# sotelo/parrot

Measured on AMD Instinct MI355X. Metric: acoustic feature frames/sec (train fwd+bwd+allreduce+clip/Adam), higher is better.
Workload: dtype f32; 1 GPU; BASELINE configs[1]: 2-layer attention-GRU decoder, h=1024, batch=64 per GPU, T_enc=200, T_dec=800, fp32; cell=gru, layers=2, hidden=1024, batch_per_gpu=64, global_batch=64, T_enc=200, T_dec=800, parallelism=dp1, params=13919212

## Files before the change

include/parrot_hip.h:

```cpp
#ifndef PARROT_HIP_H
#define PARROT_HIP_H

#include <stddef.h>
#include <stdint.h>

#ifdef __cplusplus
extern "C" {
#endif

#define PARROT_ERR_BADARG 10001
#define PARROT_ERR_UNSUPPORTED 10002

#define PARROT_NORM_EPS 1e-5f
#define PARROT_MAX_LAYERS 3

const char* parrot_hip_version(void);

int parrot_profile_begin(void);
long long parrot_profile_end(double* total_us, double* flops, double* bytes);
long long parrot_profile_end2(double* total_us, double* flops, double* bytes, double* plain4);

#define PARROT_PRECISION_F32 0
#define PARROT_PRECISION_BF16 1
#define PARROT_PRECISION_BF16X3 2
// ... 130 lines not shown
    const float* Wg_f[PARROT_MAX_LAYERS];
    const float* Wc_f[PARROT_MAX_LAYERS];
    const float* Wg_r[PARROT_MAX_LAYERS];
    const float* Wc_r[PARROT_MAX_LAYERS];
    int* att_sup;
    float* persist_ws;
    long long persist_ws_floats;
    float* dh_b[PARROT_MAX_LAYERS];
    float* dhup_b[PARROT_MAX_LAYERS];
    float* dw_b;
    float* dw0_b;
    float* dhup_c[PARROT_MAX_LAYERS];
    float* dw_c;
    float* dw0_c;
    void* dG16[PARROT_MAX_LAYERS];
} ParrotDecoderDesc;

long long parrot_decoder_persist_floats(const ParrotDecoderDesc* desc);
int parrot_decoder_is_persistent(void* plan);
int parrot_decoder_schedule(void* plan);
int parrot_decoder_backward_tick(void* plan);
long long parrot_decoder_trace(void* plan, int which, long long* out, long long cap);
long long parrot_decoder_trace_jobs(void* plan, int which, long long* out, long long cap);
int parrot_decoder_status(void* plan);

int parrot_decoder_create(const ParrotDecoderDesc* desc, void** plan);
int parrot_decoder_writes_bf16_grads(void* plan);
int parrot_decoder_seq_fwd(void* plan, void* stream);
int parrot_decoder_seq_bwd(void* plan, void* stream);
int parrot_decoder_destroy(void* plan);

#define PARROT_READOUT_MAX_SEG 4
typedef struct ParrotReadoutComposedDesc {
    long long M;
    long long ws_floats;
    int nseg, R, O, zero_rows;
    int slice_rows, nbias;
    int K[PARROT_READOUT_MAX_SEG];
    int ldx[PARROT_READOUT_MAX_SEG];
    int lddx[PARROT_READOUT_MAX_SEG];
    int ldwr, ldwo, ldp, lddp;
    int ldgwr, ldgwo;
    const float* x[PARROT_READOUT_MAX_SEG];
    const float* Wr; const float* Wo;
    const float* rb[PARROT_READOUT_MAX_SEG];
    const float* bo;
// ... 196 lines not shown
```

parrot_amd/_lib.py:

```python
from __future__ import annotations

import ctypes as C
import os

from .utils import env_str

_HERE = os.path.dirname(os.path.abspath(__file__))
LIB_PATH = os.path.join(_HERE, "libparrot_hip.so")

MAX_LAYERS = 3

c_float_p = C.c_void_p


class HipLibraryMissing(RuntimeError):
    pass


class HipCallError(RuntimeError):
    pass


class GruSeqDesc(C.Structure):
    _fields_ = [
# ... 170 lines not shown
    "parrot_label_gather": (_i, [C.POINTER(LabelTablesDesc), _vp]),
    "parrot_label_segsum_ws_floats": (C.c_longlong, [_ll, _i, _i]),
    "parrot_label_segsum": (_i, [C.POINTER(LabelTablesDesc), _vp, _ll, _vp]),
    "parrot_gru_seq_create": (_i, [C.POINTER(GruSeqDesc), C.POINTER(C.c_void_p)]),
    "parrot_gru_seq_fwd": (_i, [_vp, _vp]),
    "parrot_gru_seq_bwd": (_i, [_vp, _vp]),
    "parrot_gru_seq_destroy": (_i, [_vp]),
    "parrot_gru_seq_route": (_i, [_vp, C.POINTER(C.c_int)]),
    "parrot_gru_seq_rowwise_supported": (_i, [_i, _i, _i, _i]),
    "parrot_lstm_seq_create": (_i, [C.POINTER(LstmSeqDesc), C.POINTER(C.c_void_p)]),
    "parrot_lstm_seq_fwd": (_i, [_vp, _vp]),
    "parrot_lstm_seq_bwd": (_i, [_vp, _vp]),
    "parrot_lstm_seq_destroy": (_i, [_vp]),
    "parrot_gmm_attention_fwd": (_i, [_vp] * 10 + [_i] * 6 + [_f] * 4 + [_vp]),
    "parrot_gmm_attention_bwd": (_i, [_vp] * 10 + [_i] * 6 + [_f, _vp]),
    "parrot_decoder_create": (_i, [C.POINTER(DecoderDesc), C.POINTER(C.c_void_p)]),
    "parrot_decoder_persist_floats": (C.c_longlong, [C.POINTER(DecoderDesc)]),
    "parrot_decoder_is_persistent": (_i, [_vp]),
    "parrot_decoder_schedule": (_i, [_vp]),
    "parrot_decoder_backward_tick": (_i, [_vp]),
    "parrot_decoder_writes_bf16_grads": (_i, [_vp]),
    "parrot_decoder_trace": (C.c_longlong, [_vp, _i, C.POINTER(C.c_longlong), C.c_longlong]),
    "parrot_decoder_trace_jobs": (C.c_longlong, [_vp, _i, C.POINTER(C.c_longlong), C.c_longlong]),
    "parrot_decoder_seq_fwd": (_i, [_vp, _vp]),
    "parrot_decoder_seq_bwd": (_i, [_vp, _vp]),
    "parrot_decoder_destroy": (_i, [_vp]),
    "parrot_readout_composed_ws_floats": (C.c_longlong, [C.POINTER(ReadoutComposedDesc)]),
    "parrot_readout_composed_fwd": (_i, [C.POINTER(ReadoutComposedDesc), _vp, _vp]),
    "parrot_readout_composed_bwd": (_i, [C.POINTER(ReadoutComposedDesc), _vp, _vp]),
    "parrot_sample_create": (_i, [C.POINTER(SampleDesc), C.POINTER(C.c_void_p)]),
    "parrot_sample_persist_floats": (C.c_longlong, [C.POINTER(SampleDesc)]),
    "parrot_sample_is_persistent": (_i, [_vp]),
    "parrot_sample_is_bf16": (_i, [_vp]),
    "parrot_sample_plan_pieces_dry": (_i, [C.POINTER(SampleDesc), _i, C.POINTER(C.c_int)]),
    "parrot_sample_plan_digest_dry": (_i, [C.POINTER(SampleDesc), _i, C.POINTER(C.c_ulonglong)]),
    "parrot_sample_status": (_i, [_vp]),
    "parrot_sample_stops_early": (_i, [_vp]),
    "parrot_sample_steps_run": (_i, [_vp, C.POINTER(C.c_int)]),
    "parrot_decoder_status": (_i, [_vp]),
    "parrot_sample_run": (_i, [_vp, _vp]),
    "parrot_sample_destroy": (_i, [_vp]),
    "parrot_plan_last_error": (_i, [_vp]),
    "parrot_sumsq": (_i, [_vp, _sz, _vp, _vp]),
    "parrot_tile_weights": (_i, [_vp, _i, _i, _i, _vp, _i, _i, _vp]),
    "parrot_tile_weights_bf16": (_i, [_vp, _i, _i, _i, _vp, _i, _i, _vp]),
    "parrot_set_gemm_precision": (_i, [_i]),
# ... 54 lines not shown
```

parrot_amd/build.py:

```python
from __future__ import annotations

import hashlib
import os
import subprocess
import sys
from concurrent.futures import ThreadPoolExecutor

from .utils import env_str

HERE = os.path.dirname(os.path.abspath(__file__))
CSRC = os.path.join(HERE, "csrc")
OUT = os.path.join(HERE, "libparrot_hip.so")
OBJDIR = os.path.join(CSRC, "build")
ARCH = "gfx950"

SOURCES = ["skinny.hip", "biggemm.hip", "attention.hip", "elementwise.hip", "quantize.hip",
           "plans.hip", "plans_decode.hip", "capi.hip", "samplernn.hip", "persist.hip", "sr_persist.hip", "rowgru.hip", "trainops.hip", "readout.hip",
           "gmmcost.hip", "labeltables.hip"]
EXTRA_FLAGS = {"quantize.hip": ["-ffp-contract=off"]}
if env_str("PARROT_PM_DEPTH"):
    EXTRA_FLAGS["persist.hip"] = ["-DPM_DEPTH=" + env_str("PARROT_PM_DEPTH")]


def _hipcc() -> str:
    for cand in (os.environ.get("HIPCC"), "/opt/rocm/bin/hipcc", "hipcc"):
        if cand and (os.path.isabs(cand) and os.path.exists(cand) or not os.path.isabs(cand)):
            return cand
    return "hipcc"


def _digest(paths) -> str:
    h = hashlib.sha256()
    for p in sorted(paths):
        with open(p, "rb") as f:
            h.update(p.encode())
            h.update(f.read())
    return h.hexdigest()


def build(force: bool = False, verbose: bool = True, timers: bool = False) -> str:
    global OUT, OBJDIR
    if timers:
# ... 41 lines not shown
```

parrot_amd/csrc/plans.hip:

```cpp
#include "pm_builder.h"
#include "switches.h"

namespace {

struct GruSeqPlan : PlanBase {
    ParrotGruSeqDesc d;

    bool rowwise = false;
    int reason = PARROT_GRU_ROUTE_SHAPE;
    int waves = 4;
    float* tiled = nullptr;
    ~GruSeqPlan() override {
        if (tiled) (void)hipFree(tiled);
    }
    int launch_path(int why) {
        rowwise = false;
        reason = why;
        return 0;
    }
    int setup_rowwise() {
        if (!rowgru_supported(d.T, d.B, d.H, d.nchain)) return launch_path(PARROT_GRU_ROUTE_SHAPE);
        if (env_int("PARROT_GRU_ROWWISE", 1) == 0) return launch_path(PARROT_GRU_ROUTE_SWITCH);
        for (int ch = 0; ch < d.nchain; ++ch)
            if (!d.Wg[ch] || !d.Wc[ch] || ((uintptr_t)d.Wg[ch] & 15) || ((uintptr_t)d.Wc[ch] & 15))
// ... 178 lines not shown
    bool persist_ok = false;
    PmProgram pm_prog;

    ~DecoderPlan() override {
        if (att_flags && !flags_fake) (void)hipFree(att_flags);
        if (bwd_flags && !flags_fake) (void)hipFree(bwd_flags);
    }

    int run(int which, hipStream_t s) override {
        BgPrecisionScope precision(d.bf16 ? 1 : -1);
        return PlanBase::run(which, s);
    }

    int enqueue(int which, hipStream_t s) override {
        BgPrecisionScope precision(d.bf16 ? 1 : -1);
        if (which == 0 && persist_ok) return pm_launch(pm_prog, s);
        if (schedule == 3) return which == 0 ? fwd_skew(s) : bwd_skew(s);
        if (which == 1 && bwd_hetero && (schedule == 0 || schedule == 5)) return bwd8(s);
        if (schedule == 5) return which == 0 ? fwd5(s) : bwd(s);
        if (schedule == 7) return which == 0 ? fwd7(s) : bwd(s);
        return which == 0 ? fwd(s) : bwd(s);
    }

    int trace(int which, std::vector<TraceRec>& out, std::vector<TraceJob>* jobs_out = nullptr) {
        if (persist_ok || (schedule != 0 && schedule < 5) || d.layer_norm) return PARROT_ERR_UNSUPPORTED;
        Tracer tr;
        g_tracer = &tr;
        const int rc = enqueue(which, nullptr);
        g_tracer = nullptr;
        out.swap(tr.recs);
        if (jobs_out) jobs_out->swap(tr.jobs);
        return rc;
    }

    int krows(int l) const { return d.H + d.E + l * d.H; }
    float* dctx(float* of_l0, float* of_upper, int l, int t) const {
        const size_t BE = (size_t)d.B * d.E;
        return l == 0 ? of_l0 + (size_t)t * BE : of_upper + (size_t)(t + 1) * BE;
    }
    SkSeg fseg(const float* A, int lda, int l, int g, int r0, int K, int ldw) const {
        if (tiled) {
            const float* Wt = g == 0 ? d.Wg_f[l] : d.Wc_f[l];
            if (d.bf16) return sk_seg(A, lda, Wt + (size_t)(r0 >> 5) * 256, (krows(l) >> 5) * 256, K, 3);
            return sk_seg(A, lda, Wt + (size_t)(r0 >> 4) * 256, (krows(l) >> 4) * 256, K, 2);
        }
        const float* W = g == 0 ? d.Wg[l] : d.Wc[l];
        return sk_seg(A, lda, W + (size_t)r0 * ldw, ldw, K, 0);
    }
    SkSeg rseg(const float* A, int l, int g, int r0, int ldw) const {
        if (tiled) {
            const float* Wt = g == 0 ? d.Wg_r[l] : d.Wc_r[l];
            if (d.bf16) return sk_seg(A, ldw, Wt + (size_t)(r0 >> 4) * (ldw >> 5) * 256, (ldw >> 5) * 256, ldw, 3);
            return sk_seg(A, ldw, Wt + (size_t)(r0 >> 4) * (ldw >> 4) * 256, (ldw >> 4) * 256, ldw, 2);
        }
// ... 926 lines not shown
int parrot_decoder_schedule(void* plan) { return plan ? static_cast<DecoderPlan*>(plan)->schedule : -1; }
int parrot_decoder_backward_tick(void* plan) { return plan ? (static_cast<DecoderPlan*>(plan)->bwd_hetero ? 8 : (static_cast<DecoderPlan*>(plan)->bwd_fused ? 7 : 0)) : -1; }
int parrot_decoder_writes_bf16_grads(void* plan) {
    const DecoderPlan* p = static_cast<const DecoderPlan*>(plan);
    if (!p || !p->bwd_fused) return 0;
    for (int l = 0; l < p->d.L; ++l)
        if (!p->d.dG16[l]) return 0;
    return 1;
}
long long parrot_decoder_trace_jobs(void* plan, int which, long long* out, long long cap) { PH_ENTRY();
    if (!plan || which < 0 || which > 1) return -PARROT_ERR_BADARG;
    std::vector<TraceRec> recs;
    std::vector<TraceJob> jobs;
    const int rc = static_cast<DecoderPlan*>(plan)->trace(which, recs, &jobs);
    if (rc != 0) return -(long long)rc;
    const long long n = (long long)jobs.size();
    if (out)
        for (long long i = 0; i < n && i < cap; ++i) {
            out[6 * i] = jobs[i].launch; out[6 * i + 1] = jobs[i].job; out[6 * i + 2] = jobs[i].M;
            out[6 * i + 3] = jobs[i].N; out[6 * i + 4] = jobs[i].Kmax_seg_sum; out[6 * i + 5] = jobs[i].epi;
        }
    return n;
}
long long parrot_decoder_trace(void* plan, int which, long long* out, long long cap) { PH_ENTRY();
    if (!plan || which < 0 || which > 1) return -PARROT_ERR_BADARG;
    std::vector<TraceRec> recs;
    const int rc = static_cast<DecoderPlan*>(plan)->trace(which, recs);
    if (rc != 0) return -(long long)rc;
    const long long n = (long long)recs.size();
    if (out)
        for (long long i = 0; i < n && i < cap; ++i) {
            out[5 * i] = recs[i].launch; out[5 * i + 1] = recs[i].job; out[5 * i + 2] = recs[i].kind;
            out[5 * i + 3] = recs[i].lo; out[5 * i + 4] = recs[i].hi;
        }
    return n;
}

int parrot_decoder_seq_fwd(void* plan, void* stream) { PH_ENTRY(); return static_cast<PlanBase*>(plan)->run(0, (hipStream_t)stream); }
int parrot_decoder_seq_bwd(void* plan, void* stream) { PH_ENTRY(); return static_cast<PlanBase*>(plan)->run(1, (hipStream_t)stream); }
int parrot_decoder_destroy(void* plan) { PH_ENTRY();
    delete static_cast<PlanBase*>(plan);
    return 0;
}

int parrot_plan_last_error(void* plan) { PH_ENTRY(); return plan ? static_cast<PlanBase*>(plan)->last_error : PARROT_ERR_BADARG; }

// ... 2 lines not shown
```

parrot_amd/csrc/plans_common.h:

```cpp
#pragma once
#include <stdlib.h>
#include <string.h>
#include <algorithm>
#include <array>
#include <memory>
#include <new>
#include <vector>
#include "../../include/parrot_hip.h"
#include "attention.h"
#include "biggemm.h"
#include "elementwise.h"
#include "persist.h"
#include "rowgru.h"
#include "skinny.h"

namespace {


struct PlanBase {
    int last_error = 0;
    int use_graph = 0;
    hipGraphExec_t exec[2] = {nullptr, nullptr};
    hipStream_t cap_stream = nullptr;
    virtual ~PlanBase() {
// ... 23 lines not shown
            e = hipGraphInstantiate(&exec[which], graph, nullptr, nullptr, 0);
            hipGraphDestroy(graph);
            if (e != hipSuccess) {
                exec[which] = nullptr;
                return note((int)e);
            }
        }
        return note((int)hipGraphLaunch(exec[which], s));
    }
    int note(int rc) {
        if (rc != 0 && last_error == 0) last_error = rc;
        return rc;
    }
};

#define PL_TRY(x)                \
    do {                         \
        const int rc__ = (x);    \
        if (rc__ != 0) return rc__; \
    } while (0)

struct TraceRec { long long launch, job, kind, lo, hi; };
struct TraceJob { long long launch, job, M, N, Kmax_seg_sum, epi; };
struct Tracer {
    std::vector<TraceRec> recs;
    std::vector<TraceJob> jobs;
    long long launch = -1;
    void begin() { ++launch; }
    void mat(const void* p, long long rows, long long cols, long long ld, int kind, int job, int elt = 4) {
        if (!p || rows < 1 || cols < 1) return;
        const long long base = (long long)(uintptr_t)p;
        if (ld == cols) { recs.push_back({launch, job, kind, base, base + rows * cols * elt}); return; }
        for (long long r = 0; r < rows; ++r) recs.push_back({launch, job, kind, base + r * ld * elt, base + (r * ld + cols) * elt});
    }
    void sk_job(const SkJob& j, int id) {
        long long ks = 0;
        for (int q = 0; q < j.nseg; ++q) ks += j.seg[q].K;
        jobs.push_back({launch, id, j.M, j.N, ks, j.epi});
        for (int q = 0; q < j.nseg; ++q)
            mat(j.seg[q].A, j.M, j.seg[q].K, j.seg[q].lda, (j.wait_flag && (j.wait_all || q == j.nseg - 1)) ? 3 : 0, id);
        mat(j.add, j.M, j.N, j.ld_add, 0, id);
        const int H = j.H;
        switch (j.epi) {
            case SK_EPI_LINEAR:
                mat(j.out, j.M, j.N, j.ldo, j.accumulate ? 2 : 1, id);
                if (j.ksplit > 1) mat(j.o1, j.M, j.N, j.ldo1, j.ldo2 ? 2 : 1, id);
                if (j.ksplit > 2) mat(j.kout2, j.M, j.N, j.ldo1, 1, id);
                if (j.ksplit > 3) mat(j.kout3, j.M, j.N, j.ldo1, 1, id);
                break;
            case SK_EPI_GRU_GATES:
                mat(j.e0, j.M, H, j.lde0, 0, id); mat(j.o1, j.M, H, j.ldo1, 1, id); mat(j.o2, j.M, H, j.ldo2, 1, id);
// ... 37 lines not shown
    }
    void chain(const LstmStateBwdChain& c, int B, int H, int id) {
        mat(c.dh, B, H, H, 0, id); mat(c.dh2, B, H, H, 0, id); mat(c.dh3, B, H, H, 0, id); mat(c.dh4, B, H, H, 0, id);
        mat(c.dh5, B, H, H, 0, id); mat(c.dh6, B, H, H, 0, id);
        mat(c.gates, B, 4 * H, 4 * H, 0, id);
        mat(c.c_prev, B, H, H, 0, id); mat(c.c_new, B, H, H, 0, id);
        mat(c.dc, B, H, H, 2, id); mat(c.dP, B, 4 * H, 4 * H, 1, id);
        mat(c.dP16, B, 4 * H, 4 * H, 1, id, 2);
    }
};
thread_local Tracer* g_tracer = nullptr;
enum { TRACE_JOB_ATT = 100, TRACE_JOB_CHAIN = 200 };

int launch_jobs(const SkJob* jobs, int n, hipStream_t s, int full_wgs = 0, int force_tile = 0, int force_wide = 0) {
    SkLaunch L;
    PL_TRY(sk_make_launch(L, jobs, n));
    L.force_wide = force_wide;
    if (g_tracer) {
        g_tracer->begin();
        for (int q = 0; q < n; ++q) {
            if (jobs[q].wait_flag) return PARROT_ERR_BADARG;
            g_tracer->sk_job(jobs[q], q);
        }
        return 0;
    }
    L.full_wgs = full_wgs;
    L.force_tile = force_tile;
    return sk_launch(L, s);
}

int traced_att_fwd_launch(const AttFwdArgs& att, hipStream_t s) {
    if (g_tracer) {
        g_tracer->begin();
        g_tracer->att_fwd(att, TRACE_JOB_ATT);
        return 0;
    }
    return att_fwd_launch(att, s);
}

int launch_jobs_att(const SkJob* jobs, int n, const AttFwdArgs& att, hipStream_t s, int full_wgs = 0) {
    if (n < 1) return traced_att_fwd_launch(att, s);
    SkLaunch L;
    PL_TRY(sk_make_launch(L, jobs, n));
    if (g_tracer) {
        g_tracer->begin();
        g_tracer->att_fwd(att, TRACE_JOB_ATT);
// ... 129 lines not shown
```

parrot_amd/csrc/skinny.h:

```cpp
#pragma once
#include "common.h"

#ifndef SK_NWAVES
#define SK_NWAVES 8
#endif
enum { SK_MAXSEG = 5, SK_MAXJOB = 9, SK_NW = SK_NWAVES, SK_THREADS = SK_NW * 64 };

enum SkEpi {
    SK_EPI_LINEAR = 0,
    SK_EPI_GRU_GATES = 1,
    SK_EPI_GRU_CAND = 2,
    SK_EPI_BWD_RH = 3,
    SK_EPI_LSTM = 4,
};

enum SkAct { SK_ACT_NONE = 0, SK_ACT_RELU = 1, SK_ACT_TANH = 2, SK_ACT_SIGMOID = 3 };

struct SkSeg {
    const float* A;
    const float* B;
    int lda, ldb, K, b_kcontig;
};

struct SkJob {
    SkSeg seg[SK_MAXSEG];
    int nseg, M, N, epi;
    int act, accumulate, H, aligned;
    const float* bias;
    const float* add;
// ... 2 lines not shown
    const float* e1;
    float* o1;
    float* o2;
    const float* mask;
    int ld_add, ldo, lde0, lde1, ldo1, ldo2, wait_all, ksplit;
    float* kout2;
    float* kout3;
    const unsigned* wait_flag;
    unsigned wait_target;
    int colmode;
};

struct SkLaunch {
    SkJob job[SK_MAXJOB];
    int njobs, zmode;
    int tile_end[SK_MAXJOB];
    int force_tile;
    int force_wide;
    int full_wgs;
};

int sk_launch(const SkLaunch& L, hipStream_t stream);
void sk_prepare(const SkLaunch& Lin, SkLaunch& L, dim3& grid, size_t& lds, int& mbnb);
struct AttFwdArgs;
int sk_launch_att(const SkLaunch& L, const AttFwdArgs& att, hipStream_t stream);
struct AttBwdArgs;
struct GruStateBwdArgs;
int sk_launch_bwd_hetero(const SkLaunch& L, const AttBwdArgs* att, const GruStateBwdArgs& sa, int l0_chain, hipStream_t stream);
struct LstmStateBwdArgs;
int sk_launch_bwd_fused(const SkLaunch& L, const AttBwdArgs* att, const LstmStateBwdArgs& sa, int l0_chain,
                        unsigned* const* flags, hipStream_t stream);
int sk_zero_words_launch(unsigned* p, int n, hipStream_t stream);
void sk_profile_begin();
long long sk_profile_end(double* total_us, double* flops, double* bytes);
long long sk_profile_end2(double* total_us, double* flops, double* bytes, double* plain);

static inline SkSeg sk_seg(const float* A, int lda, const float* B, int ldb, int K, int b_kcontig) {
    SkSeg s;
    s.A = A; s.B = B; s.lda = lda; s.ldb = ldb; s.K = K; s.b_kcontig = b_kcontig;
    return s;
}
int sk_tile_weights_launch(const float* W, int rows, int cols, int ld, float* out, int mode, int lstm_H,
                           hipStream_t stream);
int sk_tile_weights_bf16_launch(const float* W, int rows, int cols, int ld, void* out, int mode, int lstm_H,
                                hipStream_t stream);
void sk_job_init(SkJob& j);
// ... 5 lines not shown
```

parrot_amd/csrc/skinny.hip:

```cpp
#include "skinny.h"
#include "att_fwd_body.h"
#include "att_bwd_body.h"
#include "elementwise.h"
#include "switches.h"

#include <stdio.h>
#include <stdlib.h>

#include <hip/hip_ext.h>
#include <string.h>
#include <type_traits>
#include <vector>

template <bool AL>
__device__ __forceinline__ f32x4 ld4k(const float* __restrict__ p, int k, int K) {
    f32x4 v = {0.f, 0.f, 0.f, 0.f};
    if (AL) {
        if (k < K) v = *reinterpret_cast<const f32x4*>(p);
    } else {
#pragma unroll
        for (int u = 0; u < 4; ++u)
            if (k + u < K) v[u] = p[u];
    }
    return v;
// ... 130 lines not shown
        __builtin_amdgcn_s_sleep(8);
        if ((++it & 1023u) == 0 && wall_clock64() - t0 > 100000000ull) __builtin_trap();
    }
    __builtin_amdgcn_fence(__ATOMIC_ACQUIRE, "workgroup");
    asm volatile("" ::: "memory");
}
__device__ __forceinline__ __amdgpu_buffer_rsrc_t sk_rsrc(const void* p) {
    const unsigned long long a = (unsigned long long)p;
    const unsigned lo = __builtin_amdgcn_readfirstlane((unsigned)a);
    const unsigned hi = __builtin_amdgcn_readfirstlane((unsigned)(a >> 32));
    void* q = (void*)(((unsigned long long)hi << 32) | lo);
    return __builtin_amdgcn_make_buffer_rsrc(q, 0, 0x7fffffff, 0x00020000);
}

#ifdef SK_TIMERS
__constant__ unsigned long long* sk_timer_buf = nullptr;
#define SK_STAMP(i)                                                                                                  \
    do {                                                                                                             \
        if (sk_timer_buf && (threadIdx.x & 63) == 0) {                                                               \
            const size_t wg_ = blockIdx.x + (size_t)gridDim.x * (blockIdx.y + (size_t)gridDim.y * blockIdx.z);       \
            sk_timer_buf[(wg_ * 16 + (threadIdx.x >> 6)) * 8 + (i)] = wall_clock64();                                \
        }                                                                                                            \
    } while (0)
#else
#define SK_STAMP(i) do { } while (0)
#endif

__device__ __forceinline__ unsigned sk_off(int m, int ld, int c) { return __umul24((unsigned)m, (unsigned)ld) + (unsigned)c; }

template <int MB, int NB, bool FAST>
__device__ __forceinline__ void sk_body(const SkJob& job, int tile0, f32x4* red) {
    const int tid = threadIdx.x;
    const int lane = tid & 63;
    const int wave = __builtin_amdgcn_readfirstlane(tid >> 6);
    const int kk = lane >> 4, i = lane & 15;
    const int m0 = blockIdx.y * (16 * MB);
    const int M = job.M, N = job.N;
    SK_STAMP(0);
    asm volatile("" ::"s"(job.M), "s"(job.N), "s"(job.epi), "s"(job.H), "s"(job.nseg), "s"(job.accumulate), "s"(job.colmode),
                 "s"(job.bias), "s"(job.add), "s"(job.out), "s"(job.e0), "s"(job.e1), "s"(job.o1), "s"(job.ld_add),
                 "s"(job.ldo), "s"(job.lde0), "s"(job.lde1), "s"(job.ldo1), "s"(job.wait_flag), "s"(job.seg[0].A),
                 "s"(job.seg[0].B), "s"(job.seg[0].lda), "s"(job.seg[0].ldb), "s"(job.seg[0].K), "s"(job.seg[0].b_kcontig),
                 "s"(job.seg[1].A), "s"(job.seg[1].B), "s"(job.seg[1].lda), "s"(job.seg[1].ldb), "s"(job.seg[1].K));
    if (m0 >= M) return;

    f32x4 acc[MB][NB];
#pragma unroll
    for (int rb = 0; rb < MB; ++rb)
#pragma unroll
        for (int nb = 0; nb < NB; ++nb) acc[rb][nb] = (f32x4){0.f, 0.f, 0.f, 0.f};

    constexpr int NBLK = MB * NB;
    constexpr int EG = (SK_NW % NBLK == 0) ? (SK_NW / NBLK > 4 ? 4 : SK_NW / NBLK) : 1;
    constexpr int RPW = 4 / EG, EWAVES = NBLK * EG;
    const int eblk = wave % NBLK, er0 = (wave / NBLK) * RPW;
    float p_bias = 0.f, p_add[RPW], p_e0[RPW], p_e1[RPW], p_oc[RPW];
#pragma unroll
    for (int r = 0; r < RPW; ++r) p_add[r] = p_e0[r] = p_e1[r] = p_oc[r] = 0.f;
    const bool has_add = job.add != nullptr;
    if (wave < EWAVES) {
        const int rb_ = eblk / NB, tile_ = tile0 + eblk % NB;
// ... 26 lines not shown
            p_oc[r] = q_oc[sk_off(m, l_oc, c_oc)];
        }
    }

    SK_STAMP(6);
    if (FAST) {
        int cend[SK_MAXSEG], slda[SK_MAXSEG], sldb[SK_MAXSEG];
        const float* sA[SK_MAXSEG];
        const float* sB[SK_MAXSEG];
        int total = 0;
        const int csh = job.seg[0].b_kcontig == 3 ? 5 : 4;
        const bool flagged = job.wait_flag != nullptr;
        const int nsm = flagged ? job.nseg - 1 : job.nseg;
#pragma unroll
        for (int s = 0; s < SK_MAXSEG; ++s) {
            const bool on = s < nsm;
            const int ss = on ? s : 0;
            if (on) total += job.seg[ss].K >> csh;
            cend[s] = total;
            sA[s] = job.seg[ss].A; sB[s] = job.seg[ss].B; slda[s] = job.seg[ss].lda; sldb[s] = job.seg[ss].ldb;
        }
        int mrow[MB], ncl[NB], btile[NB];
#pragma unroll
        for (int rb = 0; rb < MB; ++rb) mrow[rb] = min(m0 + rb * 16 + ((lane >> 2) & 15), M - 1);
#pragma unroll
        for (int nb = 0; nb < NB; ++nb) {
            ncl[nb] = min(sk_jcol(job, tile0 + nb, i), N - 1);
            btile[nb] = min(tile0 + nb, ((N + 15) >> 4) - 1);
        }
        const int mine = (total - wave + SK_NW - 1) / SK_NW;
        const int first = wave;
        const int last = wave + (mine - 1) * SK_NW;
        constexpr int STR = SK_NW;
        auto run = [&](auto kc_tag) {
            constexpr int BM = decltype(kc_tag)::value;
            auto fetch = [&](int g, f32x4 (&a)[MB], f32x4 (&b)[NB]) {
                const float* A = sA[0];
                const float* B = sB[0];
                int lda = slda[0], ldb = sldb[0], beg = 0;
#pragma unroll
                for (int s = 0; s < SK_MAXSEG - 1; ++s) {
                    const bool nx = g >= cend[s];
                    A = nx ? sA[s + 1] : A; B = nx ? sB[s + 1] : B;
                    lda = nx ? slda[s + 1] : lda; ldb = nx ? sldb[s + 1] : ldb; beg = nx ? cend[s] : beg;
                }
                sk_fetch_fast<MB, NB, BM>(A, lda, B, ldb, (g - beg) << 4, mrow, ncl, btile, kk, a, b);
            };
            f32x4 ra[SK_DEPTH][MB], rb_[SK_DEPTH][NB];
#pragma unroll
            for (int dd = 0; dd < SK_DEPTH; ++dd) fetch(min(first + dd * STR, last), ra[dd], rb_[dd]);
            int g = first;
            const int ngroups = mine / SK_DEPTH;
            for (int gr = 0; gr < ngroups; ++gr) {
#pragma unroll
                for (int dd = 0; dd < SK_DEPTH; ++dd) {
                    sk_a_unpermute<MB>(ra[dd]);
                    sk_mma2<MB, NB>(ra[dd], rb_[dd], acc);
                    fetch(min(g + (SK_DEPTH + dd) * STR, last), ra[dd], rb_[dd]);
                }
                g += SK_DEPTH * STR;
            }
            const int rem = mine - ngroups * SK_DEPTH;
#pragma unroll
            for (int dd = 0; dd < SK_DEPTH - 1; ++dd)
                if (dd < rem) {
                    sk_a_unpermute<MB>(ra[dd]);
                    sk_mma2<MB, NB>(ra[dd], rb_[dd], acc);
                }
        };
        auto run_bf16 = [&]() {
            auto fetch = [&](int g, f32x4 (&a)[MB][2], f32x4 (&b)[NB]) {
                const float* A = sA[0];
                const float* B = sB[0];
// ... 5 lines not shown
                    lda = nx ? slda[s + 1] : lda; ldb = nx ? sldb[s + 1] : ldb; beg = nx ? cend[s] : beg;
                }
                sk_fetch_bf16<MB, NB>(A, lda, B, ldb, (g - beg) << 5, mrow, btile, a, b);
            };
            f32x4 ra[SK_DEPTH][MB][2], rb_[SK_DEPTH][NB];
#pragma unroll
            for (int dd = 0; dd < SK_DEPTH; ++dd) fetch(min(first + dd * STR, last), ra[dd], rb_[dd]);
            int g = first;
            const int ngroups = mine / SK_DEPTH;
            for (int gr = 0; gr < ngroups; ++gr) {
#pragma unroll
                for (int dd = 0; dd < SK_DEPTH; ++dd) {
                    sk_mma_bf16<MB, NB>(ra[dd], rb_[dd], acc);
                    fetch(min(g + (SK_DEPTH + dd) * STR, last), ra[dd], rb_[dd]);
                }
                g += SK_DEPTH * STR;
            }
            const int rem = mine - ngroups * SK_DEPTH;
#pragma unroll
            for (int dd = 0; dd < SK_DEPTH - 1; ++dd)
                if (dd < rem) sk_mma_bf16<MB, NB>(ra[dd], rb_[dd], acc);
        };
        SK_STAMP(1);
        if (mine > 0) {
            if (job.seg[0].b_kcontig == 3) run_bf16();
            else if (job.seg[0].b_kcontig == 2) run(std::integral_constant<int, 2>{});
            else if (job.seg[0].b_kcontig == 1) run(std::integral_constant<int, 1>{});
            else run(std::integral_constant<int, 0>{});
        }
        if (flagged) {
            __syncthreads();
            if (tid == 0) sk_wait_flag(job.wait_flag, job.wait_target);
            __syncthreads();
            const SkSeg& sg = job.seg[job.nseg - 1];
            const int ntail = sg.K >> 4;
            const __amdgpu_buffer_rsrc_t rs = sk_rsrc(sg.A);
            for (int c = wave; c < ntail; c += SK_NW) {
                f32x4 a[MB], b[NB];
#pragma unroll
                for (int rb = 0; rb < MB; ++rb)
                    a[rb] = __builtin_bit_cast(f32x4, __builtin_amdgcn_raw_buffer_load_b128(
                        rs, (unsigned)((mrow[rb] * sg.lda + (c << 4) + 4 * (lane & 3)) * 4), 0, 16 ));
#pragma unroll
                for (int nb = 0; nb < NB; ++nb)
                    b[nb] = *reinterpret_cast<const f32x4*>(sg.B + (size_t)btile[nb] * sg.ldb + ((size_t)c << 8) + (lane << 2));
                sk_a_unpermute<MB>(a);
                sk_mma2<MB, NB>(a, b, acc);
// ... 147 lines not shown

__device__ __forceinline__ int sk_find_job(const SkLaunch& L, int& bx) {
    asm volatile("" ::"s"(L.njobs), "s"(L.tile_end[0]), "s"(L.tile_end[1]), "s"(L.tile_end[2]), "s"(L.tile_end[3]),
                 "s"(L.tile_end[4]), "s"(L.tile_end[5]), "s"(L.tile_end[6]), "s"(L.tile_end[7]));
    int j = 0, beg = 0;
#pragma unroll
    for (int q = 0; q < SK_MAXJOB - 1; ++q) {
        const bool nx = q < L.njobs - 1 && bx >= L.tile_end[q];
        j = nx ? q + 1 : j;
        beg = nx ? L.tile_end[q] : beg;
    }
    bx -= beg;
    return j;
}

template <int MB, int NB, bool ZMODE>
__global__ __launch_bounds__(SK_THREADS) void sk_kernel(const SkLaunch L) {
    extern __shared__ __attribute__((aligned(16))) char sk_smem[];
    f32x4* red = reinterpret_cast<f32x4*>(sk_smem);
    int j = blockIdx.z, bx = blockIdx.x;
    if (!ZMODE) j = sk_find_job(L, bx);
    const SkJob& job = L.job[j];
    const int tile0 = bx * NB;
    if (NB > 1 || job.aligned) sk_body<MB, NB, true>(job, tile0, red);
    else sk_body<MB, 1, false>(job, tile0, red);
}

#ifndef SKA_PROJ_UNROLL
#define SKA_PROJ_UNROLL 4
#endif
template <int MB, int NB>
__global__ __launch_bounds__(SK_THREADS, 4) void ska_kernel(const SkLaunch L, const AttFwdArgs g, const int natt_x,
                                                         const int att_last) {
    extern __shared__ __attribute__((aligned(16))) char sk_smem[];
    int bx = blockIdx.x;
    asm volatile("" ::"s"(natt_x), "s"(att_last), "s"((int)gridDim.x), "s"(L.njobs), "s"(L.tile_end[0]), "s"(L.tile_end[1]),
                 "s"(L.tile_end[2]), "s"(L.tile_end[3]), "s"(L.tile_end[4]), "s"(L.tile_end[5]), "s"(L.tile_end[6]),
                 "s"(L.tile_end[7]));
    if (att_last == 1) {
        const int ngemm = (int)gridDim.x - natt_x;
        bx = bx >= ngemm ? bx - ngemm : bx + natt_x;
    }
    if (bx < natt_x) {
        if (att_last == 2 && blockIdx.y != 0) return;
        const int id = att_last == 2 ? bx : blockIdx.y * natt_x + bx;
        if (id >= g.B * g.esplit) return;
        att_fwd_block<SK_THREADS, SKA_PROJ_UNROLL>(g, id / g.esplit, id % g.esplit, reinterpret_cast<float*>(sk_smem));
        return;
    }
    bx -= natt_x;
    f32x4* red = reinterpret_cast<f32x4*>(sk_smem);
    const int j = sk_find_job(L, bx);
    const SkJob& job = L.job[j];
    const int tile0 = bx * NB;
    if (NB > 1 || job.aligned) sk_body<MB, NB, true>(job, tile0, red);
    else sk_body<MB, 1, false>(job, tile0, red);
}

template <int MB, int NB>
__global__ __launch_bounds__(ATTB_THREADS) void skb_kernel(const SkLaunch L, const AttBwdArgs g, const GruStateBwdArgs sa,
                                                           const int att_rows, const int l0_chain, const int nlead,
                                                           const int nlead_x, const int rpb) {
    extern __shared__ __attribute__((aligned(16))) char sk_smem[];
    int bx = blockIdx.x;
    asm volatile("" ::"s"(att_rows), "s"(l0_chain), "s"(nlead), "s"(nlead_x), "s"(rpb), "s"(L.njobs), "s"(L.tile_end[0]),
                 "s"(L.tile_end[1]), "s"(L.tile_end[2]), "s"(L.tile_end[3]), "s"(L.tile_end[4]), "s"(L.tile_end[5]),
                 "s"(L.tile_end[6]), "s"(L.tile_end[7]));
    if (bx < nlead_x) {
        const int id = blockIdx.y * nlead_x + bx;
        if (id >= nlead) return;
        att_state_bwd_block(g, sa, att_rows, l0_chain, id, reinterpret_cast<float*>(sk_smem), rpb);
        return;
    }
    if (threadIdx.x >= SK_THREADS) return;
    bx -= nlead_x;
    f32x4* red = reinterpret_cast<f32x4*>(sk_smem);
    const int j = sk_find_job(L, bx);
    const SkJob& job = L.job[j];
    const int tile0 = bx * NB;
    if (NB > 1 || job.aligned) sk_body<MB, NB, true>(job, tile0, red);
    else sk_body<MB, 1, false>(job, tile0, red);
}

namespace {
__global__ __launch_bounds__(256) void sk_zero_words_kernel(unsigned* p, int n) {
    for (int i = blockIdx.x * 256 + threadIdx.x; i < n; i += gridDim.x * 256) p[i] = 0u;
}
}
int sk_zero_words_launch(unsigned* p, int n, hipStream_t stream) {
    if (!p || n < 1) return PH_ERR_BADARG;
    hipLaunchKernelGGL(sk_zero_words_kernel, dim3(n > 4096 ? 16 : 1), dim3(256), 0, stream, p, n);
    return (int)hipGetLastError();
}

void sk_job_init(SkJob& j) { memset(&j, 0, sizeof(j)); }

void sk_finalize_job(SkJob& j) {
    int al = 1;
    for (int s = 0; s < j.nseg; ++s) {
        const SkSeg& g = j.seg[s];
        if (((uintptr_t)g.A & 15) || (g.lda & 3) || (g.K & 15)) al = 0;
        if (g.b_kcontig && (((uintptr_t)g.B & 15) || (g.ldb & 3))) al = 0;
        if (g.b_kcontig >= 2 && (j.N & 15)) al = 0;
        if (g.b_kcontig == 3 && (g.K & 31)) al = 0;
// ... 691 lines not shown
    }
    if (Lin.force_tile > 0) {
        const int fmb = Lin.force_tile / 10, fnb = Lin.force_tile % 10;
        if (fmb >= 1 && fmb <= 4 && (fnb == 1 || (fnb == 2 && nb2_ok)) && 16 * (fmb - 1) < maxM) {
            best_mb = fmb; best_nb = fnb;
        }
    }
    const int mb = best_mb, nb = best_nb;
    int t = 0, wmax = 0;
    bool equal = true;
    for (int q = 0; q < L.njobs; ++q) {
        const int w = ceil_div(L.tile_end[q], nb);
        if (q > 0 && w != wmax) equal = false;
        wmax = w > wmax ? w : wmax;
        t += w;
        L.tile_end[q] = t;
    }
    L.zmode = equal ? 1 : 0;
    grid_out = dim3(equal ? wmax : t, ceil_div(maxM, 16 * mb), equal ? L.njobs : 1);
    lds_out = (size_t)SK_NW * mb * nb * 64 * sizeof(f32x4);
    mbnb_out = mb * 10 + nb;
}

int sk_launch(const SkLaunch& Lin, hipStream_t stream) {
    for (int q = 0; q < Lin.njobs; ++q)
        if (Lin.job[q].wait_flag) return PH_ERR_BADARG;
    {
        int rc = 0;
        if (wk_try_launch(Lin, stream, &rc)) return rc;
        for (int q = 0; q < Lin.njobs; ++q)
            if (Lin.job[q].ksplit > 1) return PH_ERR_UNSUPPORTED;
    }
    SkLaunch L;
    dim3 grid;
    size_t lds;
    int mbnb;
    sk_prepare(Lin, L, grid, lds, mbnb);
    sk_with_tile(mbnb, [&](auto mb, auto nb) {
        constexpr int MB = decltype(mb)::value, NB = decltype(nb)::value;
        if (L.zmode) sk_enqueue<sk_kernel<MB, NB, true>, false>(L, 0, grid, dim3(SK_THREADS), lds, stream, L);
        else sk_enqueue<sk_kernel<MB, NB, false>, false>(L, 0, grid, dim3(SK_THREADS), lds, stream, L);
    });
    return (int)hipGetLastError();
}

int sk_launch_att(const SkLaunch& Lin, const AttFwdArgs& att, hipStream_t stream) {
    AttFwdArgs g = att;
    {
        const int rc = att_fwd_check(g);
        if (rc != 0) return rc;
    }
    if (Lin.njobs < 1) return att_fwd_launch(att, stream);
    {
        int rc = 0;
        if (wk_try_launch(Lin, stream, &rc, &g)) return rc;
        for (int q = 0; q < Lin.njobs; ++q)
            if (Lin.job[q].wait_flag && Lin.job[q].seg[0].b_kcontig == 3) return PH_ERR_UNSUPPORTED;
    }
    SkLaunch L;
    dim3 grid;
    size_t lds;
    int mbnb;
    sk_prepare(Lin, L, grid, lds, mbnb);
// ... 54 lines not shown
```

parrot_amd/csrc/switches.h:

```cpp
#pragma once
#include <stdlib.h>

static inline int env_int(const char* name, int dflt) {
    const char* e = getenv(name);
    return e ? atoi(e) : dflt;
}
static inline bool env_set(const char* name) { return getenv(name) != nullptr; }
static inline const char* env_str(const char* name) { return getenv(name); }

static inline int sw_att_dense() { return env_int("PARROT_ATT_DENSE", 0); }
static inline int sw_pm_dataflow(int dflt) { return env_int("PARROT_PM_DATAFLOW", dflt); }
static inline int sw_rg_waves() { return env_int("PARROT_RG_WAVES", 8); }
static inline int sw_wk() { return env_int("PARROT_WK", 1); }
static inline bool sw_pm_dump_plan() { return env_set("PARROT_PM_DUMP_PLAN"); }
```

Before: 919,200 frames/s.

## Preload skinny GEMM pointers via kernel-arg SGPRs and issue first loads at entry

Adds a hot variant of the skinny GEMM kernel. The host packs A/B base offsets, strides and clamp limits for up to three aligned jobs into 16 scalar kernel arguments, and kernarg preloading is enabled for skinny.hip. Each workgroup can then issue its first SK_DEPTH prefetches right at entry, without first reading the SkLaunch struct from memory, which is meant to hide launch-time latency in the small per-step GEMMs. It adds another kernel instantiation plus encoding limits (16-bit strides, 32-bit offsets), and the path only applies to eligible launches; it can be turned off with PARROT_SK_HOT or PARROT_SK_NO_PRELOAD.

```diff
diff --git a/include/parrot_hip.h b/include/parrot_hip.h
--- a/include/parrot_hip.h
+++ b/include/parrot_hip.h
@@ -176,6 +176,7 @@
 int parrot_decoder_backward_tick(void* plan);
 long long parrot_decoder_trace(void* plan, int which, long long* out, long long cap);
 long long parrot_decoder_trace_jobs(void* plan, int which, long long* out, long long cap);
+long long parrot_decoder_trace_hot(void* plan, int which, long long* out, long long cap);
 int parrot_decoder_status(void* plan);
 
 int parrot_decoder_create(const ParrotDecoderDesc* desc, void** plan);
diff --git a/parrot_amd/_lib.py b/parrot_amd/_lib.py
--- a/parrot_amd/_lib.py
+++ b/parrot_amd/_lib.py
@@ -216,6 +216,7 @@
     "parrot_decoder_writes_bf16_grads": (_i, [_vp]),
     "parrot_decoder_trace": (C.c_longlong, [_vp, _i, C.POINTER(C.c_longlong), C.c_longlong]),
     "parrot_decoder_trace_jobs": (C.c_longlong, [_vp, _i, C.POINTER(C.c_longlong), C.c_longlong]),
+    "parrot_decoder_trace_hot": (C.c_longlong, [_vp, _i, C.POINTER(C.c_longlong), C.c_longlong]),
     "parrot_decoder_seq_fwd": (_i, [_vp, _vp]),
     "parrot_decoder_seq_bwd": (_i, [_vp, _vp]),
     "parrot_decoder_destroy": (_i, [_vp]),
diff --git a/parrot_amd/build.py b/parrot_amd/build.py
--- a/parrot_amd/build.py
+++ b/parrot_amd/build.py
@@ -17,7 +17,10 @@
 SOURCES = ["skinny.hip", "biggemm.hip", "attention.hip", "elementwise.hip", "quantize.hip",
            "plans.hip", "plans_decode.hip", "capi.hip", "samplernn.hip", "persist.hip", "sr_persist.hip", "rowgru.hip", "trainops.hip", "readout.hip",
            "gmmcost.hip", "labeltables.hip"]
-EXTRA_FLAGS = {"quantize.hip": ["-ffp-contract=off"]}
+EXTRA_FLAGS = {"quantize.hip": ["-ffp-contract=off"],
+               "skinny.hip": ["-mllvm", "-amdgpu-kernarg-preload-count=14"]}
+if env_str("PARROT_SK_NO_PRELOAD"):
+    del EXTRA_FLAGS["skinny.hip"]
 if env_str("PARROT_PM_DEPTH"):
     EXTRA_FLAGS["persist.hip"] = ["-DPM_DEPTH=" + env_str("PARROT_PM_DEPTH")]
 
diff --git a/parrot_amd/csrc/plans.hip b/parrot_amd/csrc/plans.hip
--- a/parrot_amd/csrc/plans.hip
+++ b/parrot_amd/csrc/plans.hip
@@ -224,7 +224,8 @@
         return which == 0 ? fwd(s) : bwd(s);
     }
 
-    int trace(int which, std::vector<TraceRec>& out, std::vector<TraceJob>* jobs_out = nullptr) {
+    int trace(int which, std::vector<TraceRec>& out, std::vector<TraceJob>* jobs_out = nullptr,
+              std::vector<long long>* hot_out = nullptr) {
         if (persist_ok || (schedule != 0 && schedule < 5) || d.layer_norm) return PARROT_ERR_UNSUPPORTED;
         Tracer tr;
         g_tracer = &tr;
@@ -232,6 +233,7 @@
         g_tracer = nullptr;
         out.swap(tr.recs);
         if (jobs_out) jobs_out->swap(tr.jobs);
+        if (hot_out) hot_out->swap(tr.hot);
         return rc;
     }
 
@@ -1204,6 +1206,17 @@
         }
     return n;
 }
+long long parrot_decoder_trace_hot(void* plan, int which, long long* out, long long cap) { PH_ENTRY();
+    if (!plan || which < 0 || which > 1) return -PARROT_ERR_BADARG;
+    std::vector<TraceRec> recs;
+    std::vector<long long> hot;
+    const int rc = static_cast<DecoderPlan*>(plan)->trace(which, recs, nullptr, &hot);
+    if (rc != 0) return -(long long)rc;
+    const long long n = (long long)hot.size() / TRACE_HOT_ROW;
+    if (out)
+        for (long long i = 0; i < n * TRACE_HOT_ROW && i < cap * TRACE_HOT_ROW; ++i) out[i] = hot[i];
+    return n;
+}
 long long parrot_decoder_trace(void* plan, int which, long long* out, long long cap) { PH_ENTRY();
     if (!plan || which < 0 || which > 1) return -PARROT_ERR_BADARG;
     std::vector<TraceRec> recs;
diff --git a/parrot_amd/csrc/plans_common.h b/parrot_amd/csrc/plans_common.h
--- a/parrot_amd/csrc/plans_common.h
+++ b/parrot_amd/csrc/plans_common.h
@@ -69,11 +69,30 @@
 
 struct TraceRec { long long launch, job, kind, lo, hi; };
 struct TraceJob { long long launch, job, M, N, Kmax_seg_sum, epi; };
+enum { TRACE_HOT_ROW = 14 + SK_HOTW };
 struct Tracer {
     std::vector<TraceRec> recs;
     std::vector<TraceJob> jobs;
+    std::vector<long long> hot;
     long long launch = -1;
     void begin() { ++launch; }
+    void sk_hot(const SkLaunch& Lin) {
+        SkLaunch L;
+        dim3 grid;
+        size_t lds;
+        int mbnb;
+        sk_prepare(Lin, L, grid, lds, mbnb);
+        unsigned w[SK_HOTW];
+        sk_hot_block(L, mbnb, w);
+        for (int q = 0; q < L.njobs; ++q) {
+            const SkJob& j = L.job[q];
+            const SkSeg& g = j.seg[0];
+            const long long row[14] = {launch, q, L.zmode, mbnb, j.M, j.N, (long long)(uintptr_t)g.A, (long long)(uintptr_t)g.B,
+                                       g.lda, g.ldb, g.K, g.b_kcontig, j.aligned, j.nseg};
+            hot.insert(hot.end(), row, row + 14);
+            for (int i = 0; i < SK_HOTW; ++i) hot.push_back((long long)w[i]);
+        }
+    }
     void mat(const void* p, long long rows, long long cols, long long ld, int kind, int job, int elt = 4) {
         if (!p || rows < 1 || cols < 1) return;
         const long long base = (long long)(uintptr_t)p;
@@ -157,6 +176,9 @@
             if (jobs[q].wait_flag) return PARROT_ERR_BADARG;
             g_tracer->sk_job(jobs[q], q);
         }
+        L.full_wgs = full_wgs;
+        L.force_tile = force_tile;
+        g_tracer->sk_hot(L);
         return 0;
     }
     L.full_wgs = full_wgs;
diff --git a/parrot_amd/csrc/skinny.h b/parrot_amd/csrc/skinny.h
--- a/parrot_amd/csrc/skinny.h
+++ b/parrot_amd/csrc/skinny.h
@@ -4,7 +4,8 @@
 #ifndef SK_NWAVES
 #define SK_NWAVES 8
 #endif
-enum { SK_MAXSEG = 5, SK_MAXJOB = 9, SK_NW = SK_NWAVES, SK_THREADS = SK_NW * 64 };
+enum { SK_MAXSEG = 5, SK_MAXJOB = 9, SK_NW = SK_NWAVES, SK_THREADS = SK_NW * 64,
+       SK_HOTW = 14, SK_HOTJ = 3 };
 
 enum SkEpi {
     SK_EPI_LINEAR = 0,
@@ -53,6 +54,7 @@
 
 int sk_launch(const SkLaunch& L, hipStream_t stream);
 void sk_prepare(const SkLaunch& Lin, SkLaunch& L, dim3& grid, size_t& lds, int& mbnb);
+bool sk_hot_block(const SkLaunch& L, int mbnb, unsigned* w);
 struct AttFwdArgs;
 int sk_launch_att(const SkLaunch& L, const AttFwdArgs& att, hipStream_t stream);
 struct AttBwdArgs;
diff --git a/parrot_amd/csrc/skinny.hip b/parrot_amd/csrc/skinny.hip
--- a/parrot_amd/csrc/skinny.hip
+++ b/parrot_amd/csrc/skinny.hip
@@ -176,21 +176,89 @@
             sk_timer_buf[(wg_ * 16 + (threadIdx.x >> 6)) * 8 + (i)] = wall_clock64();                                \
         }                                                                                                            \
     } while (0)
+#define SK_CLOCK() wall_clock64()
+#define SK_STAMP_AT(i, t)                                                                                            \
+    do {                                                                                                             \
+        if (sk_timer_buf && (threadIdx.x & 63) == 0) {                                                               \
+            const size_t wg_ = blockIdx.x + (size_t)gridDim.x * (blockIdx.y + (size_t)gridDim.y * blockIdx.z);       \
+            sk_timer_buf[(wg_ * 16 + (threadIdx.x >> 6)) * 8 + (i)] = (t);                                           \
+        }                                                                                                            \
+    } while (0)
 #else
 #define SK_STAMP(i) do { } while (0)
+#define SK_CLOCK() 0ull
+#define SK_STAMP_AT(i, t) do { (void)(t); } while (0)
 #endif
 
+typedef const __attribute__((address_space(1))) f32x4* SkGlobalVec;
+struct SkHotSeg {
+    unsigned long long A, B;
+    int lda, ldb, mlast, tlast, k0;
+};
+template <int MB, int NB>
+__device__ __forceinline__ void sk_fetch_hot(const SkHotSeg& hs, int kc, const int (&mrow)[MB], const int (&btile)[NB],
+                                             f32x4 (&a)[MB], f32x4 (&b)[NB]) {
+#pragma unroll
+    for (int rb = 0; rb < MB; ++rb)
+        a[rb] = *reinterpret_cast<SkGlobalVec>(hs.A + 4ull * ((size_t)mrow[rb] * hs.lda + kc + 4 * (threadIdx.x & 3)));
+#pragma unroll
+    for (int nb = 0; nb < NB; ++nb)
+        b[nb] = *reinterpret_cast<SkGlobalVec>(hs.B + 4ull * ((size_t)btile[nb] * hs.ldb + ((size_t)(kc >> 4) << 8) +
+                                                              ((threadIdx.x & 63) << 2)));
+}
+#define SK_HOT_PARAMS                                                                                                 \
+    const unsigned h0, const unsigned h1, const unsigned h2, const unsigned h3, const unsigned h4, const unsigned h5,  \
+        const unsigned h6, const unsigned h7, const unsigned h8, const unsigned h9, const unsigned h10,               \
+        const unsigned h11, const unsigned h12, const unsigned h13, const unsigned h14, const unsigned h15
+#define SK_HOT_ARGS h0, h1, h2, h3, h4, h5, h6, h7, h8, h9, h10, h11, h12, h13, h14, h15
+__device__ __forceinline__ bool sk_hot_decode(SK_HOT_PARAMS, int j, SkHotSeg& s) {
+    const unsigned a = j == 0 ? h4 : (j == 1 ? h7 : h10);
+    const unsigned b = j == 0 ? h5 : (j == 1 ? h8 : h11);
+    const unsigned c = j == 0 ? h6 : (j == 1 ? h9 : h12);
+    const unsigned long long base = ((unsigned long long)h1 << 32) | h0;
+    s.A = base + ((unsigned long long)a << 4);
+    s.B = base + ((unsigned long long)b << 4);
+    s.lda = (int)(c & 0xffffu);
+    s.ldb = (int)((c >> 16) << 8);
+    s.mlast = (int)(h2 & 0xffffffu);
+    s.k0 = (int)(h2 >> 24);
+    s.tlast = (int)(h3 & 0xffffu);
+    (void)h13; (void)h14; (void)h15;
+    return j < SK_HOTJ && ((h3 >> (16 + j)) & 1u) != 0;
+}
+
 __device__ __forceinline__ unsigned sk_off(int m, int ld, int c) { return __umul24((unsigned)m, (unsigned)ld) + (unsigned)c; }
 
-template <int MB, int NB, bool FAST>
-__device__ __forceinline__ void sk_body(const SkJob& job, int tile0, f32x4* red) {
+template <bool FIRST, typename A, typename B>
+__device__ __forceinline__ auto sk_pick(A* a, B* b) {
+    if constexpr (FIRST) return a;
+    else return b;
+}
+template <int MB, int NB, bool FAST, bool HOT = false>
+__device__ __forceinline__ void sk_body(const SkJob& job, int tile0, f32x4* red, const SkHotSeg& hs) {
+    static_assert(!HOT || FAST, "the hot block feeds the fast path only");
     const int tid = threadIdx.x;
     const int lane = tid & 63;
     const int wave = __builtin_amdgcn_readfirstlane(tid >> 6);
     const int kk = lane >> 4, i = lane & 15;
     const int m0 = blockIdx.y * (16 * MB);
     const int M = job.M, N = job.N;
-    SK_STAMP(0);
+    f32x4 ha[HOT ? SK_DEPTH : 1][MB], hb[HOT ? SK_DEPTH : 1][NB];
+    int hrow[MB], htile[NB];
+    if constexpr (HOT) {
+        const unsigned long long t_entry = SK_CLOCK();
+#pragma unroll
+        for (int rb = 0; rb < MB; ++rb) hrow[rb] = min(m0 + rb * 16 + ((lane >> 2) & 15), hs.mlast);
+#pragma unroll
+        for (int nb = 0; nb < NB; ++nb) htile[nb] = min(tile0 + nb, hs.tlast);
+#pragma unroll
+        for (int dd = 0; dd < SK_DEPTH; ++dd) sk_fetch_hot<MB, NB>(hs, (wave + dd * SK_NW) << 4, hrow, htile, ha[dd], hb[dd]);
+        const unsigned long long t_req = SK_CLOCK();
+        SK_STAMP_AT(0, t_entry);
+        SK_STAMP_AT(7, t_req);
+    } else {
+        SK_STAMP(0);
+    }
     asm volatile("" ::"s"(job.M), "s"(job.N), "s"(job.epi), "s"(job.H), "s"(job.nseg), "s"(job.accumulate), "s"(job.colmode),
                  "s"(job.bias), "s"(job.add), "s"(job.out), "s"(job.e0), "s"(job.e1), "s"(job.o1), "s"(job.ld_add),
                  "s"(job.ldo), "s"(job.lde0), "s"(job.lde1), "s"(job.ldo1), "s"(job.wait_flag), "s"(job.seg[0].A),
@@ -263,11 +331,11 @@
         }
         int mrow[MB], ncl[NB], btile[NB];
 #pragma unroll
-        for (int rb = 0; rb < MB; ++rb) mrow[rb] = min(m0 + rb * 16 + ((lane >> 2) & 15), M - 1);
+        for (int rb = 0; rb < MB; ++rb) mrow[rb] = HOT ? hrow[rb] : min(m0 + rb * 16 + ((lane >> 2) & 15), M - 1);
 #pragma unroll
         for (int nb = 0; nb < NB; ++nb) {
             ncl[nb] = min(sk_jcol(job, tile0 + nb, i), N - 1);
-            btile[nb] = min(tile0 + nb, ((N + 15) >> 4) - 1);
+            btile[nb] = HOT ? htile[nb] : min(tile0 + nb, ((N + 15) >> 4) - 1);
         }
         const int mine = (total - wave + SK_NW - 1) / SK_NW;
         const int first = wave;
@@ -287,9 +355,14 @@
                 }
                 sk_fetch_fast<MB, NB, BM>(A, lda, B, ldb, (g - beg) << 4, mrow, ncl, btile, kk, a, b);
             };
-            f32x4 ra[SK_DEPTH][MB], rb_[SK_DEPTH][NB];
-#pragma unroll
-            for (int dd = 0; dd < SK_DEPTH; ++dd) fetch(min(first + dd * STR, last), ra[dd], rb_[dd]);
+            f32x4 ra_[HOT ? 1 : SK_DEPTH][MB], rbb_[HOT ? 1 : SK_DEPTH][NB];
+            f32x4(&ra)[SK_DEPTH][MB] = *sk_pick<HOT>(&ha, &ra_);
+            f32x4(&rb_)[SK_DEPTH][NB] = *sk_pick<HOT>(&hb, &rbb_);
+            if constexpr (!HOT) {
+#pragma unroll
+                for (int dd = 0; dd < SK_DEPTH; ++dd) fetch(min(first + dd * STR, last), ra[dd], rb_[dd]);
+                SK_STAMP(7);
+            }
             int g = first;
             const int ngroups = mine / SK_DEPTH;
             for (int gr = 0; gr < ngroups; ++gr) {
@@ -341,7 +414,9 @@
                 if (dd < rem) sk_mma_bf16<MB, NB>(ra[dd], rb_[dd], acc);
         };
         SK_STAMP(1);
-        if (mine > 0) {
+        if constexpr (HOT) {
+            run(std::integral_constant<int, 2>{});
+        } else if (mine > 0) {
             if (job.seg[0].b_kcontig == 3) run_bf16();
             else if (job.seg[0].b_kcontig == 2) run(std::integral_constant<int, 2>{});
             else if (job.seg[0].b_kcontig == 1) run(std::integral_constant<int, 1>{});
@@ -535,8 +610,16 @@
     if (!ZMODE) j = sk_find_job(L, bx);
     const SkJob& job = L.job[j];
     const int tile0 = bx * NB;
-    if (NB > 1 || job.aligned) sk_body<MB, NB, true>(job, tile0, red);
-    else sk_body<MB, 1, false>(job, tile0, red);
+    if (NB > 1 || job.aligned) sk_body<MB, NB, true>(job, tile0, red, SkHotSeg{});
+    else sk_body<MB, 1, false>(job, tile0, red, SkHotSeg{});
+}
+
+template <int MB, int NB>
+__global__ __launch_bounds__(SK_THREADS) void skh_kernel(SK_HOT_PARAMS, const SkLaunch L) {
+    extern __shared__ __attribute__((aligned(16))) char sk_smem[];
+    SkHotSeg hs;
+    sk_hot_decode(SK_HOT_ARGS, (int)blockIdx.z, hs);
+    sk_body<MB, NB, true, true>(L.job[blockIdx.z], (int)blockIdx.x * NB, reinterpret_cast<f32x4*>(sk_smem), hs);
 }
 
 #ifndef SKA_PROJ_UNROLL
@@ -566,8 +649,8 @@
     const int j = sk_find_job(L, bx);
     const SkJob& job = L.job[j];
     const int tile0 = bx * NB;
-    if (NB > 1 || job.aligned) sk_body<MB, NB, true>(job, tile0, red);
-    else sk_body<MB, 1, false>(job, tile0, red);
+    if (NB > 1 || job.aligned) sk_body<MB, NB, true>(job, tile0, red, SkHotSeg{});
+    else sk_body<MB, 1, false>(job, tile0, red, SkHotSeg{});
 }
 
 template <int MB, int NB>
@@ -591,8 +674,8 @@
     const int j = sk_find_job(L, bx);
     const SkJob& job = L.job[j];
     const int tile0 = bx * NB;
-    if (NB > 1 || job.aligned) sk_body<MB, NB, true>(job, tile0, red);
-    else sk_body<MB, 1, false>(job, tile0, red);
+    if (NB > 1 || job.aligned) sk_body<MB, NB, true>(job, tile0, red, SkHotSeg{});
+    else sk_body<MB, 1, false>(job, tile0, red, SkHotSeg{});
 }
 
 namespace {
@@ -1330,6 +1413,46 @@
     mbnb_out = mb * 10 + nb;
 }
 
+bool sk_hot_block(const SkLaunch& L, int mbnb, unsigned* w) {
+    (void)mbnb;
+    memset(w, 0, SK_HOTW * sizeof(unsigned));
+    if (!sw_sk_hot() || !L.zmode || L.njobs < 1) return false;
+    const int M0 = L.job[0].M, T0 = (L.job[0].N + 15) >> 4;
+    if (T0 - 1 > 0xffff) return false;
+    bool cand[SK_HOTJ];
+    uintptr_t base = ~(uintptr_t)0;
+    for (int q = 0; q < SK_HOTJ; ++q) {
+        cand[q] = false;
+        if (q >= L.njobs) continue;
+        const SkJob& j = L.job[q];
+        const SkSeg& g = j.seg[0];
+        cand[q] = j.aligned == 1 && !j.wait_flag && g.b_kcontig == 2 && j.M == M0 && ((j.N + 15) >> 4) == T0 && g.lda >= 0 &&
+                  g.lda <= 0xffff && g.ldb >= 0 && (g.ldb & 255) == 0 && (g.ldb >> 8) <= 0xffff;
+        if (!cand[q]) continue;
+        base = (uintptr_t)g.A < base ? (uintptr_t)g.A : base;
+        base = (uintptr_t)g.B < base ? (uintptr_t)g.B : base;
+    }
+    int k0 = 255;
+    unsigned ok = 0;
+    for (int q = 0; q < SK_HOTJ; ++q) {
+        if (!cand[q]) continue;
+        const SkSeg& g = L.job[q].seg[0];
+        const uintptr_t oa = (uintptr_t)g.A - base, ob = (uintptr_t)g.B - base;
+        if ((oa & 15) || (ob & 15) || (oa >> 4) > 0xffffffffull || (ob >> 4) > 0xffffffffull) continue;
+        w[4 + 3 * q] = (unsigned)(oa >> 4);
+        w[5 + 3 * q] = (unsigned)(ob >> 4);
+        w[6 + 3 * q] = (unsigned)g.lda | ((unsigned)(g.ldb >> 8) << 16);
+        ok |= 1u << q;
+        k0 = (g.K >> 4) < k0 ? (g.K >> 4) : k0;
+    }
+    if (!ok) return false;
+    w[0] = (unsigned)((unsigned long long)base & 0xffffffffull);
+    w[1] = (unsigned)((unsigned long long)base >> 32);
+    w[2] = (unsigned)(M0 - 1) | ((unsigned)k0 << 24);
+    w[3] = (unsigned)(T0 - 1) | (ok << 16);
+    return L.njobs <= SK_HOTJ && ok == (1u << L.njobs) - 1u && k0 >= SK_DEPTH * SK_NW;
+}
+
 int sk_launch(const SkLaunch& Lin, hipStream_t stream) {
     for (int q = 0; q < Lin.njobs; ++q)
         if (Lin.job[q].wait_flag) return PH_ERR_BADARG;
@@ -1344,9 +1467,14 @@
     size_t lds;
     int mbnb;
     sk_prepare(Lin, L, grid, lds, mbnb);
+    unsigned h[SK_HOTW];
+    const bool hot = sk_hot_block(L, mbnb, h);
     sk_with_tile(mbnb, [&](auto mb, auto nb) {
         constexpr int MB = decltype(mb)::value, NB = decltype(nb)::value;
-        if (L.zmode) sk_enqueue<sk_kernel<MB, NB, true>, false>(L, 0, grid, dim3(SK_THREADS), lds, stream, L);
+        if (hot)
+            sk_enqueue<skh_kernel<MB, NB>, false>(L, 0, grid, dim3(SK_THREADS), lds, stream, h[0], h[1], h[2], h[3], h[4], h[5], h[6],
+                                                  h[7], h[8], h[9], h[10], h[11], h[12], h[13], 0u, 0u, L);
+        else if (L.zmode) sk_enqueue<sk_kernel<MB, NB, true>, false>(L, 0, grid, dim3(SK_THREADS), lds, stream, L);
         else sk_enqueue<sk_kernel<MB, NB, false>, false>(L, 0, grid, dim3(SK_THREADS), lds, stream, L);
     });
     return (int)hipGetLastError();
diff --git a/parrot_amd/csrc/switches.h b/parrot_amd/csrc/switches.h
--- a/parrot_amd/csrc/switches.h
+++ b/parrot_amd/csrc/switches.h
@@ -11,5 +11,6 @@
 static inline int sw_att_dense() { return env_int("PARROT_ATT_DENSE", 0); }
 static inline int sw_pm_dataflow(int dflt) { return env_int("PARROT_PM_DATAFLOW", dflt); }
 static inline int sw_rg_waves() { return env_int("PARROT_RG_WAVES", 8); }
+static inline int sw_sk_hot() { return env_int("PARROT_SK_HOT", 1); }
 static inline int sw_wk() { return env_int("PARROT_WK", 1); }
 static inline bool sw_pm_dump_plan() { return env_set("PARROT_PM_DUMP_PLAN"); }
```

Result: no change. 928,100 frames/s (median of 6 runs) (+1.0%).
